# OpenDrift/opendrift

Measured on AMD Instinct MI355X. Metric: particle-steps/sec (RK4, 3D interp), higher is better.
Workload: dtype f64; 1 GPU; C3: OceanDrift 3D, synthetic ROMS-shaped z-level grid 1024x1024x12 (u,v,w,K), RK4 + vertical_mixing(60 s) + vertical_advection; particles_per_gpu=10000000, particles_total=10000000, stage_math=fast, spin_up_steps=200, block_every=0, inputs=resident in HBM, parallelism=particle-sharded x1, field block broadcast once per time level

## Files before the change

### include/odrift.h

```cpp
#ifndef ODRIFT_H
#define ODRIFT_H
#include <stdint.h>

#ifdef __cplusplus
extern "C" {
#endif

typedef struct odr_ctx odr_ctx;
typedef struct odr_particles odr_particles;

typedef enum {
  ODR_OK = 0,
  ODR_ERR_INVALID = -1,
  ODR_ERR_HIP = -2,
  ODR_ERR_CAPACITY = -3,
  ODR_ERR_STATE = -4
} odr_status;

enum {
  ODR_VAR_X_SEA_WATER_VELOCITY = 0,
  ODR_VAR_Y_SEA_WATER_VELOCITY = 1,
  ODR_VAR_X_WIND = 2,
  ODR_VAR_Y_WIND = 3,
  ODR_VAR_UPWARD_SEA_WATER_VELOCITY = 4,
// ... 243 lines not shown
  double layer_thick, particle_diameter, dissolved_diameter, diameter_uncertainty, desorption_depth, desorption_depth_uncert,
      resuspension_depth, resuspension_depth_uncert, resuspension_critvel;
} odr_radio_setup;
typedef struct odr_radio odr_radio;
int odr_radio_create(odr_ctx *ctx, const odr_radio_setup *setup, odr_radio **out);
int odr_radio_counts(odr_ctx *ctx, odr_radio *radio, int64_t *counts49, int reset);
int odr_radio_destroy(odr_ctx *ctx, odr_radio *radio);
int odr_radio_speciation(odr_ctx *ctx, odr_particles *p, odr_radio *radio, int specie_slot, int diameter_slot, int32_t conc3_var,
                         double dt_seconds, int rng_mode, const double *u1, const double *u2, const double *diameter_noise,
                         const double *depth_noise, uint64_t step);
int odr_radio_terminal_velocity(odr_ctx *ctx, odr_particles *p, int diameter_slot, int density_slot);
int odr_radio_resuspend(odr_ctx *ctx, odr_particles *p, odr_radio *radio, int specie_slot, int diameter_slot, int rng_mode,
                        const double *diameter_noise, const double *depth_noise, uint64_t step);
int odr_particles_count_status(odr_ctx *ctx, odr_particles *p, int32_t status_code, int64_t *n);
int odr_particles_remap_status(odr_ctx *ctx, odr_particles *p, int32_t from_code, int32_t to_code);
int odr_deactivate(odr_ctx *ctx, odr_particles *p, const uint8_t *mask_host, int32_t status_code);
int odr_deactivate_outside(odr_ctx *ctx, odr_particles *p, double west, double east, double south, double north,
                           int32_t status_code);
int odr_compact(odr_ctx *ctx, odr_particles *p, int64_t *n_active);
int odr_scan_status(odr_ctx *ctx, odr_particles *p, int64_t *n_kept, uint64_t *status_flags);
int odr_scan_status_begin(odr_ctx *ctx, odr_particles *p);
int odr_scan_status_end(odr_ctx *ctx, odr_particles *p, int64_t *n_kept, uint64_t *status_flags);
int odr_ctx_guard_next_vmix(odr_ctx *ctx, int on);
int odr_compact_apply(odr_ctx *ctx, odr_particles *p, int64_t *n_active);
int odr_sort_particles(odr_ctx *ctx, odr_particles *p, int32_t source_id);
int odr_sort_particles_ex(odr_ctx *ctx, odr_particles *p, int32_t source_id, int keep_environment);
int odr_particles_tile_stats(odr_ctx *ctx, odr_particles *p, uint64_t *out4);
int odr_particles_step_layout_stats(odr_ctx *ctx, odr_particles *p, uint64_t *out2);
int odr_particles_step_onlevel_stats(odr_ctx *ctx, odr_particles *p, uint64_t *out1);
int odr_particles_vmix_layout_stats(odr_ctx *ctx, odr_particles *p, uint64_t *out3);
int odr_particles_vmix_kplane_stats(odr_ctx *ctx, odr_particles *p, uint64_t *out2);
int odr_particles_vmix_window_stats(odr_ctx *ctx, odr_particles *p, uint64_t *out3);
int odr_particles_vmix_skip_stats(odr_ctx *ctx, odr_particles *p, uint64_t *out2);
int odr_reduce_scalars(odr_ctx *ctx, odr_particles *p, double wind_drift_depth, double *out16);
int odr_ctx_set_step_reduce(odr_ctx *ctx, int on, double wind_drift_depth, int relative_wind);
int odr_reduce_local(odr_ctx *ctx, odr_particles *p, double wind_drift_depth, int relative_wind, double *out16);
int odr_reduce_install(odr_ctx *ctx, odr_particles *p, const double *in16);
int odr_reduce_unpin(odr_ctx *ctx);

int odr_ctx_set_position_class(odr_ctx *ctx, int f32);
int odr_source_set_coordinate_dtype(odr_ctx *ctx, int32_t source_id, int x_is_float32, int y_is_float32);

#define ODR_COMM_ID_BYTES 256
int odr_device_count(int32_t *n);
int odr_comm_unique_id(uint8_t *id );
int odr_comm_init(odr_ctx *ctx, const uint8_t *id, int32_t rank, int32_t nranks);
int odr_comm_info(int32_t *rank, int32_t *nranks, uint64_t *id_hash, int32_t *rccl_version, uint64_t *collectives);
int odr_comm_destroy(void);
int odr_allreduce_scalars(odr_ctx *ctx, double *values, int32_t n, int32_t op);
int odr_comm_allgather_begin(odr_ctx *ctx, const double *row, int32_t n, int32_t from_scan);
int odr_comm_allgather_end(odr_ctx *ctx, double *rows );
int odr_comm_broadcast_bytes(odr_ctx *ctx, void *buf, int64_t nbytes, int32_t root);
int odr_comm_barrier(odr_ctx *ctx);
int odr_block_broadcast(odr_ctx *ctx, int32_t source_id, int32_t slot, double t_epoch, int nvars, const int32_t *var_ids,
                        const void *const *data, const int32_t *var_nz, int ny, int nx, const double *xy8, int32_t root);

int odr_timer_begin(odr_ctx *ctx);
int odr_timer_end(odr_ctx *ctx, float *ms);

enum {
  ODR_HIST_LON = 1000, ODR_HIST_LAT, ODR_HIST_Z, ODR_HIST_STATUS, ODR_HIST_MOVING, ODR_HIST_AGE_SECONDS,
  ODR_HIST_WIND_DRIFT_FACTOR, ODR_HIST_CURRENT_DRIFT_FACTOR, ODR_HIST_TERMINAL_VELOCITY,
  ODR_HIST_PROPERTY0 = 2000
};
typedef struct odr_history odr_history;
int odr_history_create(odr_ctx *ctx, int64_t n_trajectories, int32_t n_times, int32_t nvars,
// ... 97 lines not shown
```

### opendrift_amd/_abi.py

```python
import ctypes as C
import os

HERE = os.path.dirname(os.path.abspath(__file__))
LIB_PATH = os.environ.get('ODR_LIB') or os.path.join(HERE, 'libodrift_hip.so')

NVAR = 26
VARIABLES = {
    'x_sea_water_velocity': 0, 'y_sea_water_velocity': 1, 'x_wind': 2, 'y_wind': 3,
    'upward_sea_water_velocity': 4, 'ocean_vertical_diffusivity': 5,
    'sea_surface_wave_stokes_drift_x_velocity': 6, 'sea_surface_wave_stokes_drift_y_velocity': 7,
    'land_binary_mask': 8, 'sea_floor_depth_below_sea_level': 9, 'sea_surface_height': 10,
    'horizontal_diffusivity': 11, 'sea_surface_wave_significant_height': 12,
    'sea_surface_wave_period_at_variance_spectral_density_maximum': 13,
    'ocean_mixed_layer_thickness': 14,
    'sea_water_temperature': 15, 'sea_water_salinity': 16,
    'sea_ice_area_fraction': 17, 'sea_ice_x_velocity': 18, 'sea_ice_y_velocity': 19,
    'sea_surface_swell_wave_to_direction': 20,
    'sea_surface_swell_wave_peak_period_from_variance_spectral_density': 21,
    'sea_surface_swell_wave_significant_height': 22, 'sea_surface_wind_wave_to_direction': 23,
    'sea_surface_wind_wave_mean_period': 24, 'sea_surface_wind_wave_significant_height': 25,
}
VARIABLE_NAMES = {v: k for k, v in VARIABLES.items()}
PROJ_LATLONG, PROJ_STERE_EQUIT_SPHERE, PROJ_STERE_POLAR = 0, 1, 2
PROJ_MERC, PROJ_LCC = 4, 5
# ... 149 lines not shown
    'odr_particles_count_status': [_vp, _vp, C.c_int32, _i64p],
    'odr_particles_remap_status': [_vp, _vp, C.c_int32, C.c_int32],
    'odr_deactivate': [_vp, _vp, _P(C.c_uint8), C.c_int32],
    'odr_deactivate_outside': [_vp, _vp, C.c_double, C.c_double, C.c_double, C.c_double, C.c_int32],
    'odr_compact': [_vp, _vp, _i64p],
    'odr_vmix_set_profile_levels': [_vp, C.c_int32],
    'odr_ctx_set_position_class': [_vp, C.c_int],
    'odr_source_set_coordinate_dtype': [_vp, C.c_int32, C.c_int, C.c_int],
    'odr_device_count': [_P(C.c_int32)],
    'odr_comm_unique_id': [_P(C.c_uint8)],
    'odr_comm_init': [_vp, _P(C.c_uint8), C.c_int32, C.c_int32],
    'odr_comm_info': [_P(C.c_int32), _P(C.c_int32), _P(C.c_uint64), _P(C.c_int32), _P(C.c_uint64)],
    'odr_comm_destroy': [],
    'odr_allreduce_scalars': [_vp, _dp, C.c_int32, C.c_int32],
    'odr_comm_allgather_begin': [_vp, _dp, C.c_int32, C.c_int32],
    'odr_comm_allgather_end': [_vp, _dp],
    'odr_comm_broadcast_bytes': [_vp, _vp, C.c_int64, C.c_int32],
    'odr_comm_barrier': [_vp],
    'odr_block_broadcast': [_vp, C.c_int32, C.c_int32, C.c_double, C.c_int, _ip, _P(_vp), _ip, C.c_int, C.c_int, _dp, C.c_int32],
    'odr_scan_status': [_vp, _vp, _i64p, _P(C.c_uint64)],
    'odr_scan_status_begin': [_vp, _vp],
    'odr_scan_status_end': [_vp, _vp, _i64p, _P(C.c_uint64)],
    'odr_ctx_guard_next_vmix': [_vp, C.c_int],
    'odr_compact_apply': [_vp, _vp, _i64p],
    'odr_sort_particles': [_vp, _vp, C.c_int32],
    'odr_sort_particles_ex': [_vp, _vp, C.c_int32, C.c_int],
    'odr_particles_tile_stats': [_vp, _vp, _P(C.c_uint64)],
    'odr_particles_step_layout_stats': [_vp, _vp, _P(C.c_uint64)],
    'odr_particles_step_onlevel_stats': [_vp, _vp, _P(C.c_uint64)],
    'odr_particles_vmix_layout_stats': [_vp, _vp, _P(C.c_uint64)],
    'odr_particles_vmix_kplane_stats': [_vp, _vp, _P(C.c_uint64)],
    'odr_particles_vmix_window_stats': [_vp, _vp, _P(C.c_uint64)],
    'odr_particles_vmix_skip_stats': [_vp, _vp, _P(C.c_uint64)],
    'odr_reduce_scalars': [_vp, _vp, C.c_double, _dp],
    'odr_ctx_set_step_reduce': [_vp, C.c_int, C.c_double, C.c_int],
    'odr_reduce_local': [_vp, _vp, C.c_double, C.c_int, _dp],
    'odr_reduce_install': [_vp, _vp, _dp],
    'odr_reduce_unpin': [_vp],
    'odr_timer_begin': [_vp],
    'odr_timer_end': [_vp, _fp],
    'odr_sgrid_create': [_vp, C.c_int32, C.c_int32, C.c_int32, _dp, _dp, C.c_double, _dp, _dp, C.c_int32, _P(_vp)],
    'odr_sgrid_destroy': [_vp, _vp],
    'odr_sgrid_download_zrho': [_vp, _vp, _dp],
    'odr_sgrid_zslice': [_vp, _vp, _vp, C.c_int, C.c_int, C.c_int32, _dp, C.c_int32, _P(_vp), _dp],
    'odr_history_create': [_vp, C.c_int64, C.c_int32, C.c_int32, _ip, _P(_vp)],
    'odr_history_destroy': [_vp, _vp],
    'odr_history_set_id_base': [_vp, _vp, C.c_int64],
    'odr_history_record': [_vp, _vp, _vp, C.c_int32, C.c_int, C.c_int],
    'odr_history_flush': [_vp, _vp, C.c_int32, C.c_int32],
    'odr_history_wait': [_vp, _vp],
    'odr_history_host_ptr': [_vp, _vp, C.c_int32, _P(_fp), _P(C.c_int32)],
    'odr_history_reset': [_vp, _vp],
    'odr_history_minmax': [_vp, _vp, C.c_int32, _dp, _dp],
    'odr_density_map': [_vp, C.c_int64, C.c_int32] + [_vp] * 5 + [C.c_int32, C.c_int32, _dp, C.c_int32, _dp, _dp, _dp, _dp],
    'odr_density_last_kernel_ms': [_vp, _fp],
    'odr_density_map_proj': [_vp, C.c_int64, C.c_int32] + [_vp] * 5 + [C.c_int32, _P(ProjDesc), C.c_int32, _dp, C.c_int32, _dp, C.c_int64, _dp, _dp, _dp],
    'odr_species_layer_map': [_vp, C.c_int64, C.c_int32] + [_vp] * 4 + [_P(ProjDesc), C.c_int32, _dp, C.c_int32, _dp, C.c_int32, _dp, C.c_int32, _dp],
    'odr_conc_last_kernel_ms': [_vp, _fp],
    'odr_proj_extent': [_vp, _P(ProjDesc), C.c_int64, _vp, _vp, _dp],
    'odr_proj_grid_lonlat': [_vp, _P(ProjDesc), C.c_int32, _dp, C.c_int32, _dp, _dp, _dp],
    'odr_box_smooth': [_vp, C.c_int64, C.c_int32, C.c_int32, C.c_int32, _dp, _dp],
    'odr_ftle_map': [_vp, _P(ProjDesc), C.c_int32, C.c_int32, _dp, _dp, C.c_double, C.c_double, _vp, _vp, _fp, _dp],
    'odr_ftle_last_kernel_ms': [_vp, _fp],
    'odr_geod_inverse': [_vp, C.c_int64, _dp, _dp, _dp, _dp, _dp, _dp, _dp],
    'odr_trajectory_lengths': [_vp, C.c_int64, C.c_int32, _vp, _vp, C.c_double, _dp, _dp, _dp],
    'odr_trajectory_lengths_last_kernel_ms': [_vp, _fp],
# ... 71 lines not shown
```

### opendrift_amd/csrc/odr_host.h

```cpp
#pragma once
#include <hip/hip_runtime.h>

#include <algorithm>
#include <cmath>
#include <cstdarg>
#include <cstdio>
#include <cstdlib>
#include <cstring>
#include <initializer_list>
#include <string>
#include <vector>

#include "../../include/odrift.h"
#include "odr_kernels.hip.h"

using namespace odr;

#include <chrono>
struct SlowSpan {
  const char *what;
  std::chrono::steady_clock::time_point t0;
  static double limit() { static const double v = getenv("ODR_SLOW_CALLS") ? atof(getenv("ODR_SLOW_CALLS")) : 0.0; return v; }
  explicit SlowSpan(const char *w) : what(w) { if (limit() > 0) t0 = std::chrono::steady_clock::now(); }
  ~SlowSpan() {
// ... 99 lines not shown
  float *env[NVAR];
  float *altenv[NVAR];
  float *aux[9];
  float *altaux[9];
  bool profiles_f32 = false;
  unsigned aux_user = 0;
  bool kmember_on = false;
  float *aux_snap[9];
  long long aux_snap_cap[9];
  double *dead64[3];
  int *deadi32[2];
  unsigned *bcount;
  unsigned *wcount;
  unsigned long long wcount_epoch;
  long long wcount_n;
  void *scratch;
  size_t scratch_bytes;
  unsigned long long epoch;
  unsigned long long status_epoch, scan_epoch;
  long long scan_kept;
  float env_cval[NVAR];
  long long env_cn[NVAR];
  bool env_cok[NVAR];
  bool external;
  unsigned *wg_tab, *wg_list;
  unsigned long long *wg_total, *wg_stats;
  long long wg_cap, wg_grid, wg_n, wg_list_cap;
  unsigned long long wg_launches;
  unsigned long long step_launches[3];
  unsigned long long vmix_launches[3];
  unsigned long long vmix_kplane[2];
  unsigned long long vmix_window[2];
  unsigned long long vmix_tiled;
  unsigned long long *vmix_redone;
  double *z_keep;
  long long z_keep_n;
  bool z_truncated;
  int wg_sid;
  bool wg_valid;
  unsigned wg_src_gen;
};

static inline unsigned nblk(long long n) { return (unsigned)((n + BLOCK - 1) / BLOCK); }

static inline PView view(const odr_particles *p) {
  PView v;
  v.n = p->n;
  v.lon = p->d64[0]; v.lat = p->d64[1]; v.z = p->d64[2]; v.plon = p->d64[3]; v.plat = p->d64[4];
  v.slon = p->d64[5]; v.slat = p->d64[6];
  v.id = p->i32[0]; v.status = p->i32[1]; v.moving = p->i32[2];
  v.wdf = p->f32[0]; v.cdf = p->f32[1]; v.tv = p->f32[2]; v.age = p->f32[3];
  for (int k = 0; k < NVAR; ++k) v.env[k] = p->env[k];
  for (int k = 0; k < 9; ++k) v.aux[k] = p->aux[k];
  v.ice = p->ice_kind; v.pad = 0;
  v.rank = p->rank_on && p->rank ? p->rank : nullptr;
  return v;
}

static inline EnvGroupDesc env_bind_out(const EnvGroupDesc &G0, const PView &v) {
  EnvGroupDesc G = G0;
  for (int k = 0; k < MAXG; ++k) G.out_ptr[k] = k < G.nv ? v.env[G.var[k]] : nullptr;
  return G;
}

int flush_world(odr_ctx *c);
int flush_world_init(odr_ctx *c);

// ... 169 lines not shown
```

### opendrift_amd/csrc/odr_kernels.hip.h

```cpp
#pragma once
#include <hip/hip_runtime.h>
#include <rocrand/rocrand_kernel.h>
#include "odr_field.hip.h"

namespace odr {

#ifndef ODR_BLOCK
#define ODR_BLOCK 256
#endif
constexpr int BLOCK = ODR_BLOCK;
#ifndef ODR_POLAR_WAVES
#define ODR_POLAR_WAVES 3
#endif
#ifndef ODR_POLAR_STEP_WAVES
#define ODR_POLAR_STEP_WAVES 2
#endif
#define ODR_STEP_WAVES(PROJ) ((PROJ) == PROJ_LATLONG ? ODR_LATLONG_WAVES : ((PROJ) == PROJ_EXT ? 1 : ODR_POLAR_STEP_WAVES))
#ifndef ODR_LATLONG_WAVES
#define ODR_LATLONG_WAVES 1
#endif
#define ODR_WAVES(PROJ) ((PROJ) == PROJ_LATLONG ? ODR_LATLONG_WAVES : ((PROJ) == PROJ_EXT ? 1 : ODR_POLAR_WAVES))

__device__ __forceinline__ unsigned pid_wg() {
  const unsigned nb = gridDim.x, b = blockIdx.x, per = nb >> 3, rem = nb & 7u, x = b & 7u, j = b >> 3;
  return x * per + (x < rem ? x : rem) + j;
}
__device__ __forceinline__ long long pid() { return (long long)pid_wg() * BLOCK + threadIdx.x; }

struct PView {
  long long n;
  double *lon, *lat, *z, *plon, *plat;
  double *slon, *slat;
  int *id, *status, *moving;
  float *wdf, *cdf, *tv, *age;
  float *aux[9];
  float *env[NVAR];
  int ice;
  int pad;
  const int *rank;
};

__device__ __forceinline__ int sf_species_flag(const PView &p, int sfl, long long i) {
  if ((sfl & 255) != 5) return 0;
  const int sp = (int)p.aux[(sfl >> 24) & 15][i];
  return (sp >= 0 && sp < 7 && (((sfl >> 8) >> sp) & 1)) ? 8 : 0;
}

__device__ __forceinline__ float ice_k(float A) {
  float k = __fdiv_rn(__fsub_rn(A, 0.3f), 0.5f);
  if (A < 0.3f) k = 0.f;
  if (A > 0.8f) k = 1.f;
  return k;
}
__device__ __forceinline__ float ice_stokes_factor(float A) {
  float f = __fdiv_rn(__fsub_rn(0.7f, A), 0.7f);
  if (A > 0.7f) f = 0.f;
  return f;
}
__device__ __forceinline__ float current_factor(const PView &p, long long i, float factor) {
// ... 1768 lines not shown
    Dp.wgt = vmix_per_pass(D.wgt); Dp.Kfb = vmix_per_pass(D.Kfb);
    VMixArgs A;
    A.dt = vmix_per_pass(dt); A.dt_mix_cfg = vmix_per_pass(dt_mix_cfg);
    A.mix_at_surface = mix_at_surface; A.rng_mode = rng_mode; A.sfl = sfl; A.pad = 0;
    A.huni = huni; A.seed = seed; A.step = step;
    int t;
    asm volatile("v_mbcnt_lo_u32_b32 %0, -1, 0\n\tv_mbcnt_hi_u32_b32 %0, -1, %0" : "=&v"(t));
    t += (int)wave0;
    const unsigned e = e0 + (unsigned)t;
    long long i = 0;
    bool escaped = false;
    if (e < total) {
      i = base + list[e];
      long long i1 = i;
      asm volatile("" : "+v"(i1));
      const VMixState S = vmix_load_state(p, i1);
      escaped = vmix_col_particle<NQ, TL, VM>(s, p, Dp, A, vadv, i, Kp, gsh, t, S);
    }
    if constexpr (VM::WINDOW) {
      const unsigned long long esc = __ballot(escaped);
      if (esc != 0ull) {
        if (escaped) {
          long long i2 = i;
          asm volatile("" : "+v"(i2));
          const VMixState S2 = vmix_load_state(p, i2);
          vmix_col_particle<NQ, TL, typename VM::Full>(s, p, Dp, A, vadv, i, Kp, gsh, t, S2);
          if (D.redone && (t & 63) == __ffsll((long long)esc) - 1) atomicAdd(D.redone, (unsigned long long)__popcll(esc));
        }
      }
    }
  }
}

#ifndef ODR_VWIN_WAVES
#define ODR_VWIN_WAVES 5
#endif
template <bool TL>
__device__ __forceinline__ double vmix_layer(float b00, float b01, float b10, float b11, float a00, float a01, float a10, float a11,
                                             double w00, double w01, double w10, double w11, double wgt, bool cov, double Kfb) {
  double v = (double)bilw(b00, b01, b10, b11, w00, w01, w10, w11);
  if (TL) {
    const double w = (double)bilw(a00, a01, a10, a11, w00, w01, w10, w11);
    v = __dadd_rn(__dmul_rn(v, 1 - wgt), __dmul_rn(w, wgt));
  }
  return (cov && isfinite(v)) ? v : Kfb;
}
struct VMixGrad { double gd0, gi0, gd1, gi1, gd2, gi2, dt_mix; bool uniform_z; };
__device__ __forceinline__ void vmix_terms(const VMixGrad &G, const double *gsh, int nzp, int zl, double Kl, double Kz, double Kh,
                                           double &dk_dt, double &sg) {
  const double r = 1.0 / 3, ir = 1.0 / r;
  double gK;
  if (zl == 0) gK = div_cr(Kh - Kz, G.gd0, G.gi0);
  else if (zl == nzp - 1) gK = div_cr(Kz - Kl, G.gd1, G.gi1);
  else if (G.uniform_z) gK = div_cr(Kh - Kl, G.gd2, G.gi2);
  else gK = __dadd_rn(__dadd_rn(__dmul_rn(gsh[zl], Kl), __dmul_rn(gsh[nzp + zl], Kz)), __dmul_rn(gsh[2 * nzp + zl], Kh));
  double dK = -gK;
  if (fabs(dK) < 1e-10) dK = 0;
  dk_dt = __dmul_rn(dK, G.dt_mix);
  sg = sqrt(div_cr(__dmul_rn(__dmul_rn(Kz, fabs(G.dt_mix)), 2.0), r, ir));
}
template <bool TL>
__global__ __launch_bounds__(BLOCK, ODR_VWIN_WAVES) void k_vmix_win(const DevWorld *__restrict__ W, PView p, VMixDesc D,
                                                    double dt, double dt_mix_cfg, int mix_at_surface,
                                                    int rng_mode, const double *__restrict__ huni,
                                                    unsigned long long seed, unsigned long long step,
                                                    int vadv, int sfl) {
// ... 1436 lines not shown
```

### opendrift_amd/csrc/odr_mix.hip

```cpp
#define ODR_TU_MIX 1
#include "odr_host.h"

static_assert(vmix_col_lds_bytes(3) <= 163840 / ODR_VMIX_WAVES, "k_vmix_col<3>: column, tables and offset list exceed a sixth of the LDS");

template <class VM>
static bool vmix_layout_matches(const DevSource &s, const VMixDesc &D, int nq, double dt, double dt_mix, int mix_at_surface,
                                int rng_mode, int sfl, int vadv) {
  const bool uz = s.vg_uniform != 0;
  const int ntimes = abs((int)(dt / (dt_mix * (dt > 0 ? 1.0 : (dt < 0 ? -1.0 : 0.0)))));
  return VM::proj_kind(s.proj.kind) == s.proj.kind && VM::lon_mode(s.lon_mode) == s.lon_mode &&
         VM::mod360_x(s.mod360_x) == s.mod360_x && VM::nzp(D.nzp, 4 * nq) == D.nzp && VM::uniform_z(uz) == uz &&
         VM::rng_mode(rng_mode) == rng_mode && VM::mix_at_surface(mix_at_surface) == mix_at_surface &&
         VM::sf_action(sfl & 255) == (sfl & 255) && VM::vadv(vadv) == vadv && VM::ntimes(ntimes) == ntimes &&
         VM::kstride(D.kstride, nq) == D.kstride;
}

int odr_vmix(odr_ctx *c, odr_particles *p, double t, double dt, double dt_mix, int mix_at_surface, int rng_mode,
             const double *huni, uint64_t step) {
  const bool guarded = c->guard_next_vmix != 0;
  c->guard_next_vmix = 0;
  const bool oil = c->oil_owner == p;
  const bool f32prof = p->profiles_f32;
  const int cut = c->vmix_levels;
  VMixDesc D;
  bool kplanes = !getenv("ODR_NO_KPLANE");
  const bool fast = !oil && !f32prof && cut <= 0 && !getenv("ODR_NO_FAST_PATH") && build_vmix_desc(c, t, D, kplanes);
  if (guarded && (rng_mode == ODR_RNG_HOST || !fast)) return 1;
  const int vadv = c->fuse_vadv;
  c->fuse_vadv = -1;
  c->oil_owner = nullptr;
  c->vmix_levels = 0;
  c->guarded_vmix = nullptr;
  p->status_epoch++;
  p->epoch++;
  REQUIRE(dt_mix > 0 && dt != 0, "bad time steps");
  if (!p->env[VAR_DEPTH]) return fail(ODR_ERR_STATE, "sea_floor_depth_below_sea_level has not been sampled");
// ... 22 lines not shown
  dim3 g(nblk(p->n)), b(BLOCK);
  PView v = view(p);
  unsigned long long st = (unsigned long long)step;
  if (vadv >= 0 && !p->env[VAR_W]) return fail(ODR_ERR_STATE, "upward_sea_water_velocity has not been sampled");
  struct F32ProfileClass {
    odr_ctx *c;
    bool on;
    ~F32ProfileClass() { if (on) { c->hw.f32pos &= ~2; c->dirty = true; } }
  } f32bit{c, false};
  if (f32prof) { c->hw.f32pos |= 2; c->dirty = true; f32bit.on = true; if ((rc = flush_world(c))) return rc; }
  if (cut > 0) {
    REQUIRE(cut >= 2 && cut <= 255, "odr_vmix_set_profile_levels: 2 .. 255 levels");
    if (cut < nzp) nzp = cut;
  }
  const int sfl_cut = c->seafloor | ((cut > 0 ? nzp : 0) << 16);
  if (fast) {
    if (guarded) { D.guard = c->counter + 4; c->guarded_vmix = p; c->guarded_vadv = vadv; }
    const int nq = (nzp + 3) / 4;
    const bool tl = D.ka != nullptr;
    const char *wenv = getenv("ODR_VMIX_WINDOW");
    const bool win = nzp >= 3 && nzp <= BLOCK && (wenv ? atoi(wenv) != 0 : nzp > 12);
    const bool spec = !win && (nq == 2 || nq == 3) &&
                      vmix_layout_matches<VMixC3Rec>(c->hw.src[D.sid], D, nq, dt, dt_mix, mix_at_surface, rng_mode, c->seafloor, vadv) &&
                      !getenv("ODR_NO_VMIX_SPEC");
    const bool specp = spec && vmix_layout_matches<VMixC3>(c->hw.src[D.sid], D, nq, dt, dt_mix, mix_at_surface, rng_mode, c->seafloor, vadv);
    const bool quadwin = spec && nq == 3 && !getenv("ODR_NO_VMIX_WINDOW");
    p->vmix_launches[win ? 2 : spec ? 1 : 0]++;
    p->vmix_kplane[kplanes ? 0 : 1]++;
    if (spec && nq == 3) p->vmix_window[quadwin ? 0 : 1]++;
    D.redone = quadwin ? p->vmix_redone : nullptr;
    D.skipped = p->vmix_redone + 1;
    D.noskip = getenv("ODR_NO_VMIX_SKIP") ? 1 : 0;
    if (!win) { g = dim3((unsigned)((p->n + VMIX_TILE - 1) / VMIX_TILE)); p->vmix_tiled++; }
#define VMIX_COL(NQ, VM)                                                                                          \
  do {                                                                                                            \
    const size_t l2 = vmix_col_lds_bytes(NQ);                                                                     \
    if (tl) hipLaunchKernelGGL((k_vmix_col<NQ, true, VM>), g, b, l2, c->stream, c->dw, v, D, dt, dt_mix,          \
                               mix_at_surface, rng_mode, du, c->seed, st, vadv, c->seafloor);                                  \
    else hipLaunchKernelGGL((k_vmix_col<NQ, false, VM>), g, b, l2, c->stream, c->dw, v, D, dt, dt_mix,            \
                            mix_at_surface, rng_mode, du, c->seed, st, vadv, c->seafloor);                                     \
  } while (0)
    if (win) {
      const size_t lw = (sizeof(double) + sizeof(unsigned)) * 4 * BLOCK + sizeof(double) * 4 * (size_t)nzp;
      if (tl) hipLaunchKernelGGL((k_vmix_win<true>), g, b, lw, c->stream, c->dw, v, D, dt, dt_mix, mix_at_surface, rng_mode, du,
                                 c->seed, st, vadv, c->seafloor);
      else hipLaunchKernelGGL((k_vmix_win<false>), g, b, lw, c->stream, c->dw, v, D, dt, dt_mix, mix_at_surface, rng_mode, du,
                              c->seed, st, vadv, c->seafloor);
    }
    else if (specp && nq == 2) VMIX_COL(2, VMixC3);
    else if (specp && quadwin) VMIX_COL(3, VMixC3W);
    else if (specp) VMIX_COL(3, VMixC3);
    else if (spec && nq == 2) VMIX_COL(2, VMixC3Rec);
    else if (spec && quadwin) VMIX_COL(3, VMixC3RecW);
    else if (spec) VMIX_COL(3, VMixC3Rec);
    else if (nq <= 1) VMIX_COL(1, VMixRT);
    else if (nq == 2) VMIX_COL(2, VMixRT);
    else if (nq == 3) VMIX_COL(3, VMixRT);
    else if (nq == 4) VMIX_COL(4, VMixRT);
    else if (nq <= 6) VMIX_COL(6, VMixRT);
    else if (nq <= 8) VMIX_COL(8, VMixRT);
    else if (nq <= 12) VMIX_COL(12, VMixRT);
    else VMIX_COL(16, VMixRT);
#undef VMIX_COL
  } else if (oil) {
    if (nzp <= 16) hipLaunchKernelGGL((k_vmix<16, true>), g, b, lds, c->stream, c->dw, v, t, dt, dt_mix, mix_at_surface, rng_mode, du, c->seed, st, vadv, sfl_cut, c->oil);
    else if (nzp <= 32) hipLaunchKernelGGL((k_vmix<32, true>), g, b, lds, c->stream, c->dw, v, t, dt, dt_mix, mix_at_surface, rng_mode, du, c->seed, st, vadv, sfl_cut, c->oil);
    else hipLaunchKernelGGL((k_vmix<1, true>), g, b, lds, c->stream, c->dw, v, t, dt, dt_mix, mix_at_surface, rng_mode, du, c->seed, st, vadv, sfl_cut, c->oil);
  } else if (nzp <= 16) hipLaunchKernelGGL(k_vmix<16>, g, b, lds, c->stream, c->dw, v, t, dt, dt_mix, mix_at_surface, rng_mode, du, c->seed, st, vadv, sfl_cut);
  else if (nzp <= 32) hipLaunchKernelGGL(k_vmix<32>, g, b, lds, c->stream, c->dw, v, t, dt, dt_mix, mix_at_surface, rng_mode, du, c->seed, st, vadv, sfl_cut);
  else hipLaunchKernelGGL(k_vmix<1>, g, b, lds, c->stream, c->dw, v, t, dt, dt_mix, mix_at_surface, rng_mode, du, c->seed, st, vadv, sfl_cut);
  if (!fast) p->vmix_launches[2]++;
  HIPCHK(hipGetLastError());
  return 0;
}

int odr_particles_vmix_layout_stats(odr_ctx *c, odr_particles *p, uint64_t *out3) {
  REQUIRE(c && p && out3, "NULL argument");
  for (int k = 0; k < 3; ++k) out3[k] = p->vmix_launches[k];
  return 0;
}

int odr_particles_vmix_kplane_stats(odr_ctx *c, odr_particles *p, uint64_t *out2) {
  REQUIRE(c && p && out2, "NULL argument");
  out2[0] = p->vmix_kplane[0]; out2[1] = p->vmix_kplane[1];
  return 0;
}

int odr_particles_vmix_skip_stats(odr_ctx *c, odr_particles *p, uint64_t *out2) {
  REQUIRE(c && p && out2, "NULL argument");
  unsigned long long skipped = 0;
  D2H(&skipped, p->vmix_redone + 1, sizeof skipped);
  HIPCHK(hipStreamSynchronize(c->stream));
  out2[0] = p->vmix_tiled; out2[1] = skipped;
  return 0;
}

int odr_particles_vmix_window_stats(odr_ctx *c, odr_particles *p, uint64_t *out3) {
  REQUIRE(c && p && out3, "NULL argument");
  unsigned long long redone = 0;
  D2H(&redone, p->vmix_redone, sizeof redone);
  HIPCHK(hipStreamSynchronize(c->stream));
  out3[0] = p->vmix_window[0]; out3[1] = p->vmix_window[1]; out3[2] = redone;
  return 0;
}

int odr_vmix_set_profile_levels(odr_ctx *c, int32_t n) {
  REQUIRE(n == 0 || (n >= 2 && n <= 255), "bad level count %d", n);
  c->vmix_levels = n;
  return 0;
}

int odr_vmix_wind_profile(odr_ctx *c, odr_particles *p, int model, double background_diffusivity, double dt,
                          double dt_mix, int mix_at_surface, int rng_mode, const double *huni, uint64_t step) {
  c->guard_next_vmix = 0;
  p->status_epoch++;
  p->epoch++;
  REQUIRE(model == ODR_DIFFUSIVITY_LARGE1994 || model == ODR_DIFFUSIVITY_SUNDBY1983, "Unknown diffusivity model: %d", model);
  REQUIRE(dt_mix > 0 && dt != 0, "bad time steps");
  if (!p->env[VAR_DEPTH]) return fail(ODR_ERR_STATE, "sea_floor_depth_below_sea_level has not been sampled");
  int rc;
  if ((rc = seafloor_species_slot_ok(c, p))) return rc;
  for (int v : {VAR_SSH, VAR_XWIND, VAR_YWIND, VAR_MLD})
    if ((rc = ensure_env(c, p, v))) return rc;
  if ((rc = flush_world(c))) return rc;
  if (p->n == 0) return 0;
  p->epoch++;
// ... 161 lines not shown
```

### opendrift_amd/csrc/odrift.hip

```cpp
#define ODR_TU_MISC 1
#include "odr_host.h"
#include "odr_mesh.h"

static thread_local std::string g_err;
int odr_i_fail(int code, const char *fmt, ...) {
  char buf[512];
  va_list ap;
  va_start(ap, fmt);
  vsnprintf(buf, sizeof buf, fmt, ap);
  va_end(ap);
  g_err = buf;
  return code;
}

const char *odr_last_error(void) { return g_err.c_str(); }
#define ODR_STR2(x) #x
#define ODR_STR(x) ODR_STR2(x)
const char *odr_version(void) { return "odrift-hip 0.2 (gfx950; mixing stream Philox4x32-" ODR_STR(ODR_MIX_ROUNDS) ")"; }

int odr_ctx_create(int device, uint64_t seed, odr_ctx **out) {
  REQUIRE(out, "out is NULL");
  HIPCHK(hipSetDevice(device));
  odr_ctx *c = new odr_ctx();
  c->device = device;
// ... 69 lines not shown
}

int odr_set_stream(odr_ctx *c, void *s) {
  HIPCHK(hipStreamSynchronize(c->stream));
  c->stream = s ? (hipStream_t)s : c->own_stream;
  return 0;
}

int odr_timer_begin(odr_ctx *c) {
  HIPCHK(hipEventRecord(c->ev0, c->stream));
  return 0;
}
int odr_timer_end(odr_ctx *c, float *ms) {
  HIPCHK(hipEventRecord(c->ev1, c->stream));
  HIPCHK(hipEventSynchronize(c->ev1));
  HIPCHK(hipEventElapsedTime(ms, c->ev0, c->ev1));
  return 0;
}

int odr_particles_create(odr_ctx *c, int64_t capacity, odr_particles **out) {
  REQUIRE(capacity > 0 && out, "capacity must be positive");
  HIPCHK(hipSetDevice(c->device));
  odr_particles *p = new odr_particles();
  memset(p, 0, sizeof(*p));
  p->cap = capacity;
  p->dead_cap = capacity;
  p->scan_kept = -1;
  for (int k = 0; k < 7; ++k) HIPCHK(hipMalloc((void **)&p->d64[k], sizeof(double) * (size_t)capacity));
  for (int k = 0; k < 3; ++k) HIPCHK(hipMalloc((void **)&p->i32[k], sizeof(int) * (size_t)capacity));
  for (int k = 0; k < 4; ++k) HIPCHK(hipMalloc((void **)&p->f32[k], sizeof(float) * (size_t)capacity));
  HIPCHK(hipMalloc((void **)&p->bcount, sizeof(unsigned) * (size_t)(nblk(capacity) + 1)));
  HIPCHK(hipMalloc((void **)&p->wcount, sizeof(unsigned) * (size_t)(nblk(capacity) + 1) * (BLOCK / 64)));
  p->wcount_epoch = ~0ull;
  HIPCHK(hipMalloc((void **)&p->vmix_redone, 2 * sizeof(unsigned long long)));
  HIPCHK(hipMemset(p->vmix_redone, 0, 2 * sizeof(unsigned long long)));
  *out = p;
  return 0;
}

int odr_particles_destroy(odr_ctx *c, odr_particles *p) {
  if (c->red_owner == p) c->red_owner = nullptr;
  if (c->noise_owner == p) c->noise_owner = nullptr;
  if (c->guarded_vmix == p) c->guarded_vmix = nullptr;
  if (!p) return 0;
  (void)hipStreamSynchronize(c->stream);
  auto fr = [](void *q) { if (q) (void)hipFree(q); };
  for (int k = 0; k < 7; ++k) { fr(p->d64[k]); fr(p->alt64[k]); }
  for (int k = 0; k < 3; ++k) { fr(p->i32[k]); fr(p->alti32[k]); fr(p->dead64[k]); }
  for (int k = 0; k < 4; ++k) { fr(p->f32[k]); fr(p->altf32[k]); }
  for (int k = 0; k < 2; ++k) fr(p->deadi32[k]);
  for (int k = 0; k < NVAR; ++k) { fr(p->env[k]); fr(p->altenv[k]); }
  for (int k = 0; k < 9; ++k) { fr(p->aux[k]); fr(p->altaux[k]); fr(p->aux_snap[k]); }
  fr(p->bcount);
  fr(p->wcount);
  fr(p->vmix_redone);
  fr(p->scratch);
  fr(p->rank); fr(p->rank_words); fr(p->rank_before); fr(p->rank_bsum);
  fr(p->wg_tab); fr(p->wg_total); fr(p->wg_list); fr(p->z_keep);
  delete p;
  return 0;
}

template <class T>
static int put(odr_ctx *c, T *dst, const T *src, long long n, T dflt) {
  if (src) {
    H2D(dst, src, sizeof(T) * (size_t)n);
  } else {
    std::vector<T> tmp((size_t)n, dflt);
    H2D(dst, tmp.data(), sizeof(T) * (size_t)n);
    HIPCHK(hipStreamSynchronize(c->stream));
  }
  return 0;
}

int odr_particles_append(odr_ctx *c, odr_particles *p, int64_t n, const double *lon, const double *lat,
                         const double *z, const int32_t *id, const int32_t *moving, const float *wdf,
                         const float *cdf, const float *tv) {
  p->status_epoch++;
  p->epoch++;
  REQUIRE(n >= 0 && lon && lat, "lon/lat required");
  if (p->n + n > p->cap) return fail(ODR_ERR_CAPACITY, "capacity %lld exceeded (%lld + %lld)", p->cap, p->n, (long long)n);
  if (n == 0) return 0;
  long long o = p->n;
  int rc;
  if ((rc = put<double>(c, p->d64[0] + o, lon, n, 0.0))) return rc;
  if ((rc = put<double>(c, p->d64[1] + o, lat, n, 0.0))) return rc;
  if ((rc = put<double>(c, p->d64[2] + o, z, n, 0.0))) return rc;
  if ((rc = put<double>(c, p->d64[3] + o, lon, n, 0.0))) return rc;
// ... 2400 lines not shown
```

### opendrift_amd/device.py

```python
import ctypes as C
import os

import numpy as np

from . import _abi
from ._abi import VARIABLES, check

_dp, _fp, _ip = C.POINTER(C.c_double), C.POINTER(C.c_float), C.POINTER(C.c_int32)


def _vid(v, aliases=None):
    if isinstance(v, (int, np.integer)):
        return v
    if v in VARIABLES:
        return VARIABLES[v]
    if aliases and v in aliases:
        return aliases[v]
    raise KeyError(v)


def _d(a, n=None):
    if a is None:
        return None, None
    a = np.ascontiguousarray(np.broadcast_to(np.asarray(a, dtype=np.float64), (n,)) if n is not None
# ... 1173 lines not shown
        check(self.lib.odr_particles_step_layout_stats(self.ctx.h, self.h, out))
        return dict(runtime=int(out[0]), static=int(out[1]))

    def step_onlevel_stats(self):
        import ctypes as C
        out = (C.c_uint64 * 1)()
        check(self.lib.odr_particles_step_onlevel_stats(self.ctx.h, self.h, out))
        return int(out[0])

    def vmix_layout_stats(self):
        import ctypes as C
        out = (C.c_uint64 * 3)()
        check(self.lib.odr_particles_vmix_layout_stats(self.ctx.h, self.h, out))
        return dict(runtime=int(out[0]), static=int(out[1]), other=int(out[2]))

    def vmix_kplane_stats(self):
        import ctypes as C
        out = (C.c_uint64 * 2)()
        check(self.lib.odr_particles_vmix_kplane_stats(self.ctx.h, self.h, out))
        return dict(planes=int(out[0]), records=int(out[1]))

    def vmix_window_stats(self):
        import ctypes as C
        out = (C.c_uint64 * 3)()
        check(self.lib.odr_particles_vmix_window_stats(self.ctx.h, self.h, out))
        return dict(windowed=int(out[0]), full=int(out[1]), redone=int(out[2]))

    def vmix_skip_stats(self):
        import ctypes as C
        out = (C.c_uint64 * 2)()
        check(self.lib.odr_particles_vmix_skip_stats(self.ctx.h, self.h, out))
        return dict(launches=int(out[0]), skipped=int(out[1]))

    def reduce_global(self, combine, wind_drift_depth=0.1, relative_wind=False):
        raw = np.empty(16)
        check(self.lib.odr_reduce_local(self.ctx.h, self.h, float(wind_drift_depth), int(relative_wind), raw.ctypes.data_as(_dp)))
        g = np.ascontiguousarray(combine(raw), dtype=np.float64)
        check(self.lib.odr_reduce_install(self.ctx.h, self.h, g.ctypes.data_as(_dp)))
        return g

    def reduce_local(self, wind_drift_depth=0.1, relative_wind=False):
        raw = np.empty(16)
        check(self.lib.odr_reduce_local(self.ctx.h, self.h, float(wind_drift_depth), int(relative_wind), raw.ctypes.data_as(_dp)))
        return raw

    def reduce_install(self, combined16):
        g = np.ascontiguousarray(combined16, dtype=np.float64)
        check(self.lib.odr_reduce_install(self.ctx.h, self.h, g.ctypes.data_as(_dp)))

    @staticmethod
    def reduction_dict(raw):
        keys = ['n_active', 'lon_min', 'lon_max', 'lat_min', 'lat_max', 'z_min', 'z_max', 'D_max',
                'stokes_sum_max', 'wind_speed_max', 'wdf_surface_max', 'n_surface', 'hs_max', 'tp_max']
        d = dict(zip(keys, raw))
        for k in ('lon_min', 'lat_min', 'z_min'):
            d[k] = -d[k]
        return d

    def reduce_unpin(self):
        check(self.lib.odr_reduce_unpin(self.ctx.h))

    def reduce_scalars(self, wind_drift_depth=0.1):
        out = np.empty(16)
        check(self.lib.odr_reduce_scalars(self.ctx.h, self.h, float(wind_drift_depth), out.ctypes.data_as(_dp)))
        keys = ['n_active', 'lon_min', 'lon_max', 'lat_min', 'lat_max', 'z_min', 'z_max', 'D_max',
                'stokes_sum_max', 'wind_speed_max', 'wdf_surface_max', 'n_surface', 'hs_max', 'tp_max']
# ... 334 lines not shown
```

Baseline: 11.94 billion particle-steps/s.

## Compact vertical-mixing work into a dense list of non-skipped particles

Adds a three-kernel pre-pass (ballot keep mask per tile, single-block prefix scan, list fill) that builds a compacted index list of particles that actually need vertical mixing. A new dense vmix kernel then launches over only those particles, so no wave is spent on surface particles that would be skipped. The cost is three extra launches, extra mask/list memory, a serial single-block scan, and indirect (gathered) particle access in the mixing kernel.

```diff
diff --git a/include/odrift.h b/include/odrift.h
--- a/include/odrift.h
+++ b/include/odrift.h
@@ -299,6 +299,7 @@
 int odr_particles_vmix_kplane_stats(odr_ctx *ctx, odr_particles *p, uint64_t *out2);
 int odr_particles_vmix_window_stats(odr_ctx *ctx, odr_particles *p, uint64_t *out3);
 int odr_particles_vmix_skip_stats(odr_ctx *ctx, odr_particles *p, uint64_t *out2);
+int odr_particles_vmix_dense_stats(odr_ctx *ctx, odr_particles *p, uint64_t *out2);
 int odr_reduce_scalars(odr_ctx *ctx, odr_particles *p, double wind_drift_depth, double *out16);
 int odr_ctx_set_step_reduce(odr_ctx *ctx, int on, double wind_drift_depth, int relative_wind);
 int odr_reduce_local(odr_ctx *ctx, odr_particles *p, double wind_drift_depth, int relative_wind, double *out16);
diff --git a/opendrift_amd/_abi.py b/opendrift_amd/_abi.py
--- a/opendrift_amd/_abi.py
+++ b/opendrift_amd/_abi.py
@@ -205,6 +205,7 @@
     'odr_particles_vmix_kplane_stats': [_vp, _vp, _P(C.c_uint64)],
     'odr_particles_vmix_window_stats': [_vp, _vp, _P(C.c_uint64)],
     'odr_particles_vmix_skip_stats': [_vp, _vp, _P(C.c_uint64)],
+    'odr_particles_vmix_dense_stats': [_vp, _vp, _P(C.c_uint64)],
     'odr_reduce_scalars': [_vp, _vp, C.c_double, _dp],
     'odr_ctx_set_step_reduce': [_vp, C.c_int, C.c_double, C.c_int],
     'odr_reduce_local': [_vp, _vp, C.c_double, C.c_int, _dp],
diff --git a/opendrift_amd/csrc/odr_host.h b/opendrift_amd/csrc/odr_host.h
--- a/opendrift_amd/csrc/odr_host.h
+++ b/opendrift_amd/csrc/odr_host.h
@@ -155,7 +155,10 @@
   unsigned long long vmix_kplane[2];
   unsigned long long vmix_window[2];
   unsigned long long vmix_tiled;
+  unsigned long long vmix_dense;
   unsigned long long *vmix_redone;
+  unsigned long long *vmix_mask;
+  unsigned *vmix_toff, *vmix_list;
   double *z_keep;
   long long z_keep_n;
   bool z_truncated;
diff --git a/opendrift_amd/csrc/odr_kernels.hip.h b/opendrift_amd/csrc/odr_kernels.hip.h
--- a/opendrift_amd/csrc/odr_kernels.hip.h
+++ b/opendrift_amd/csrc/odr_kernels.hip.h
@@ -21,10 +21,11 @@
 #endif
 #define ODR_WAVES(PROJ) ((PROJ) == PROJ_LATLONG ? ODR_LATLONG_WAVES : ((PROJ) == PROJ_EXT ? 1 : ODR_POLAR_WAVES))
 
-__device__ __forceinline__ unsigned pid_wg() {
-  const unsigned nb = gridDim.x, b = blockIdx.x, per = nb >> 3, rem = nb & 7u, x = b & 7u, j = b >> 3;
+__device__ __forceinline__ unsigned pid_wg_of(unsigned nb) {
+  const unsigned b = blockIdx.x, per = nb >> 3, rem = nb & 7u, x = b & 7u, j = b >> 3;
   return x * per + (x < rem ? x : rem) + j;
 }
+__device__ __forceinline__ unsigned pid_wg() { return pid_wg_of(gridDim.x); }
 __device__ __forceinline__ long long pid() { return (long long)pid_wg() * BLOCK + threadIdx.x; }
 
 struct PView {
@@ -1859,6 +1860,172 @@
   }
 }
 
+struct VMixKeep {
+  unsigned long long *mask;
+  unsigned *toff;
+  unsigned *list;
+  unsigned *hdr;
+  unsigned long long *listed;
+};
+__global__ __launch_bounds__(BLOCK) void k_vmix_keep(PView p, VMixKeep K, const unsigned long long *guard, double dt,
+                                                      double dt_mix_cfg) {
+  if (guard && *guard == 0ull) return;
+  constexpr int NW = BLOCK / 64;
+  __shared__ unsigned cnt[NW];
+  const int tid = threadIdx.x, lane = tid & 63, wave = tid >> 6;
+  const long long base = (long long)blockIdx.x * VMIX_TILE;
+  double z[VMIX_TILE_ROUNDS];
+  float dep[VMIX_TILE_ROUNDS], ssh[VMIX_TILE_ROUNDS];
+#pragma unroll
+  for (int r = 0; r < VMIX_TILE_ROUNDS; ++r) {
+    const long long e = base + r * BLOCK + tid, ec = e < p.n ? e : 0;
+    z[r] = p.z[ec]; dep[r] = p.env[VAR_DEPTH][ec]; ssh[r] = p.env[VAR_SSH][ec];
+  }
+  const double sgn = dt > 0 ? 1.0 : (dt < 0 ? -1.0 : 0.0);
+  const bool walks = abs((int)(dt / (dt_mix_cfg * sgn))) > 0;
+  unsigned mine = 0;
+#pragma unroll
+  for (int r = 0; r < VMIX_TILE_ROUNDS; ++r) {
+    const long long e = base + r * BLOCK + tid;
+    const float Zmin = __fmul_rn(-1.f, __fadd_rn(dep[r], ssh[r]));
+    const bool skip = e < p.n && z[r] == 0 && !(Zmin > 0.f);
+    if (skip && walks && __double_as_longlong(z[r]) != 0ll) p.z[e] = 0.0;
+    const unsigned long long keep = __ballot(e < p.n && !skip);
+    if (lane == 0) K.mask[(size_t)blockIdx.x * (VMIX_TILE / 64) + r * NW + wave] = keep;
+    mine += (unsigned)__popcll(keep);
+  }
+  if (lane == 0) cnt[wave] = mine;
+  __syncthreads();
+  if (tid == 0) {
+    unsigned t = 0;
+#pragma unroll
+    for (int w = 0; w < NW; ++w) t += cnt[w];
+    K.toff[blockIdx.x] = t;
+  }
+}
+constexpr int VMIX_SCAN_ROWS = 16;
+__global__ __launch_bounds__(1024) void k_vmix_keep_scan(VMixKeep K, long long ntiles, long long n,
+                                                          const unsigned long long *guard, unsigned long long *skipped) {
+  const int tid = threadIdx.x, lane = tid & 63, wv = tid >> 6;
+  if (guard && *guard == 0ull) {
+    if (tid == 0) { K.hdr[0] = 0u; K.hdr[1] = 0u; }
+    return;
+  }
+  constexpr int G = VMIX_SCAN_ROWS;
+  __shared__ unsigned wtot[G * 16];
+  unsigned carry = 0;
+  for (long long k0 = 0; k0 < ntiles; k0 += (long long)G * 1024) {
+    unsigned v[G], x[G];
+#pragma unroll
+    for (int u = 0; u < G; ++u) {
+      const long long k = k0 + (long long)u * 1024 + tid;
+      v[u] = k < ntiles ? K.toff[k] : 0u;
+    }
+#pragma unroll
+    for (int u = 0; u < G; ++u) {
+      x[u] = v[u];
+#pragma unroll
+      for (int o = 1; o < 64; o <<= 1) { const unsigned y = __shfl_up(x[u], o, 64); if (lane >= o) x[u] += y; }
+      if (lane == 63) wtot[u * 16 + wv] = x[u];
+    }
+    __syncthreads();
+    if (wv == 0) {
+#pragma unroll
+      for (int b0 = 0; b0 < G * 16; b0 += 64) {
+        const unsigned t0 = wtot[b0 + lane];
+        unsigned s = t0;
+#pragma unroll
+        for (int o = 1; o < 64; o <<= 1) { const unsigned y = __shfl_up(s, o, 64); if (lane >= o) s += y; }
+        wtot[b0 + lane] = carry + s - t0;
+        carry += __shfl(s, 63, 64);
+      }
+    }
+    __syncthreads();
+#pragma unroll
+    for (int u = 0; u < G; ++u) {
+      const long long k = k0 + (long long)u * 1024 + tid;
+      if (k < ntiles) K.toff[k] = x[u] - v[u] + wtot[u * 16 + wv];
+    }
+    __syncthreads();
+  }
+  if (tid == 0) {
+    K.hdr[0] = carry;
+    K.hdr[1] = (carry + (unsigned)BLOCK - 1u) / (unsigned)BLOCK;
+    if (skipped && (unsigned long long)n > carry) atomicAdd(skipped, (unsigned long long)n - carry);
+    if (carry) atomicAdd(K.listed, (unsigned long long)carry);
+  }
+}
+__global__ __launch_bounds__(BLOCK) void k_vmix_keep_fill(VMixKeep K, const unsigned long long *guard) {
+  if (guard && *guard == 0ull) return;
+  constexpr int NW = BLOCK / 64;
+  const int tid = threadIdx.x, lane = tid & 63;
+  const int wave = __builtin_amdgcn_readfirstlane(tid >> 6);
+  const unsigned long long *m = K.mask + (size_t)blockIdx.x * (VMIX_TILE / 64);
+  unsigned run = K.toff[blockIdx.x], off[VMIX_TILE_ROUNDS];
+  unsigned long long keep[VMIX_TILE_ROUNDS];
+#pragma unroll
+  for (int g = 0; g < VMIX_TILE / 64; ++g) {
+    const unsigned long long mg = m[g];
+    if ((g % NW) == wave) { off[g / NW] = run; keep[g / NW] = mg; }
+    run += (unsigned)__popcll(mg);
+  }
+  const unsigned long long below = (1ull << lane) - 1ull;
+  const unsigned first = (unsigned)blockIdx.x * (unsigned)VMIX_TILE;
+#pragma unroll
+  for (int r = 0; r < VMIX_TILE_ROUNDS; ++r)
+    if ((keep[r] >> lane) & 1ull) K.list[off[r] + (unsigned)__popcll(keep[r] & below)] = first + (unsigned)(r * BLOCK + tid);
+}
+__host__ __device__ constexpr size_t vmix_dense_lds_bytes(int nq) {
+  return sizeof(double) * ((size_t)(4 * nq) * BLOCK + 4 * (size_t)(4 * nq));
+}
+template <int NQ, bool TL, class VM>
+__global__ __launch_bounds__(BLOCK, ODR_VMIX_WAVES) void k_vmix_dense(const DevWorld *__restrict__ W, PView p, VMixDesc D,
+                                                      const unsigned *__restrict__ list, const unsigned *__restrict__ hdr,
+                                                      double dt, double dt_mix_cfg, int mix_at_surface,
+                                                      int rng_mode, const double *__restrict__ huni,
+                                                      unsigned long long seed, unsigned long long step,
+                                                      int vadv, int sfl) {
+  static_assert(VM::STATIC, "the dense launch exists for the static configurations");
+  constexpr int NL = 4 * NQ;
+  extern __shared__ __attribute__((aligned(16))) char smem[];
+  const int tid = threadIdx.x;
+  const DevSource &s = W->src[D.sid];
+  const int nzp = VM::nzp(D.nzp, NL);
+  double *Kp = (double *)smem;
+  double *gsh = Kp + (size_t)NL * BLOCK;
+  if (D.guard && *D.guard == 0ull) return;
+  const unsigned total = hdr[0], nbd = hdr[1];
+  if (blockIdx.x >= nbd) return;
+  const unsigned d = pid_wg_of(nbd) * BLOCK + (unsigned)tid;
+  const bool valid = d < total;
+  const long long i = list[valid ? d : 0u];
+  if (tid < nzp) {
+    gsh[tid] = s.vg_a[tid]; gsh[NL + tid] = s.vg_b[tid]; gsh[2 * NL + tid] = s.vg_c[tid];
+    gsh[3 * NL + tid] = s.zmid[tid];
+  }
+  long long i1 = i;
+  asm volatile("" : "+v"(i1));
+  const VMixState S = vmix_load_state(p, i1);
+  __syncthreads();
+  if (!valid) return;
+  VMixArgs A;
+  A.dt = dt; A.dt_mix_cfg = dt_mix_cfg; A.mix_at_surface = mix_at_surface; A.rng_mode = rng_mode; A.sfl = sfl; A.pad = 0;
+  A.huni = huni; A.seed = seed; A.step = step;
+  const bool escaped = vmix_col_particle<NQ, TL, VM>(s, p, D, A, vadv, i, Kp, gsh, tid, S);
+  if constexpr (VM::WINDOW) {
+    const unsigned long long esc = __ballot(escaped);
+    if (esc != 0ull) {
+      if (escaped) {
+        long long i2 = i;
+        asm volatile("" : "+v"(i2));
+        const VMixState S2 = vmix_load_state(p, i2);
+        vmix_col_particle<NQ, TL, typename VM::Full>(s, p, D, A, vadv, i, Kp, gsh, tid, S2);
+        if (D.redone && (tid & 63) == __ffsll((long long)esc) - 1) atomicAdd(D.redone, (unsigned long long)__popcll(esc));
+      }
+    }
+  }
+}
+
 #ifndef ODR_VWIN_WAVES
 #define ODR_VWIN_WAVES 5
 #endif
diff --git a/opendrift_amd/csrc/odr_mix.hip b/opendrift_amd/csrc/odr_mix.hip
--- a/opendrift_amd/csrc/odr_mix.hip
+++ b/opendrift_amd/csrc/odr_mix.hip
@@ -2,6 +2,8 @@
 #include "odr_host.h"
 
 static_assert(vmix_col_lds_bytes(3) <= 163840 / ODR_VMIX_WAVES, "k_vmix_col<3>: column, tables and offset list exceed a sixth of the LDS");
+static_assert(vmix_dense_lds_bytes(3) <= 163840 / ODR_VMIX_WAVES, "k_vmix_dense<3>: column and tables exceed a sixth of the LDS");
+static_assert(VMIX_TILE == 1024, "odr_particles_create sizes the keep ballots and tile counts for tiles of 1024 elements");
 
 template <class VM>
 static bool vmix_layout_matches(const DevSource &s, const VMixDesc &D, int nq, double dt, double dt_mix, int mix_at_surface,
@@ -90,6 +92,26 @@
     D.skipped = p->vmix_redone + 1;
     D.noskip = getenv("ODR_NO_VMIX_SKIP") ? 1 : 0;
     if (!win) { g = dim3((unsigned)((p->n + VMIX_TILE - 1) / VMIX_TILE)); p->vmix_tiled++; }
+    const bool dense = spec && mix_at_surface == 0 && vadv != 1 && !D.noskip && !getenv("ODR_NO_VMIX_DENSE") &&
+                       p->n <= 0xffffffffLL;
+    VMixKeep K;
+    K.mask = p->vmix_mask; K.toff = p->vmix_toff; K.list = p->vmix_list;
+    K.hdr = (unsigned *)(p->vmix_redone + 3); K.listed = p->vmix_redone + 2;
+    if (dense) {
+      hipLaunchKernelGGL(k_vmix_keep, g, b, 0, c->stream, v, K, D.guard, dt, dt_mix);
+      hipLaunchKernelGGL(k_vmix_keep_scan, dim3(1), dim3(1024), 0, c->stream, K, (long long)g.x, (long long)p->n, D.guard, D.skipped);
+      hipLaunchKernelGGL(k_vmix_keep_fill, g, b, 0, c->stream, K, D.guard);
+      g = dim3(nblk(p->n));
+      p->vmix_dense++;
+    }
+#define VMIX_DENSE(NQ, VM)                                                                                        \
+  do {                                                                                                            \
+    const size_t l2 = vmix_dense_lds_bytes(NQ);                                                                   \
+    if (tl) hipLaunchKernelGGL((k_vmix_dense<NQ, true, VM>), g, b, l2, c->stream, c->dw, v, D, K.list, K.hdr, dt, dt_mix, \
+                               mix_at_surface, rng_mode, du, c->seed, st, vadv, c->seafloor);                     \
+    else hipLaunchKernelGGL((k_vmix_dense<NQ, false, VM>), g, b, l2, c->stream, c->dw, v, D, K.list, K.hdr, dt, dt_mix, \
+                            mix_at_surface, rng_mode, du, c->seed, st, vadv, c->seafloor);                        \
+  } while (0)
 #define VMIX_COL(NQ, VM)                                                                                          \
   do {                                                                                                            \
     const size_t l2 = vmix_col_lds_bytes(NQ);                                                                     \
@@ -105,6 +127,12 @@
       else hipLaunchKernelGGL((k_vmix_win<false>), g, b, lw, c->stream, c->dw, v, D, dt, dt_mix, mix_at_surface, rng_mode, du,
                               c->seed, st, vadv, c->seafloor);
     }
+    else if (dense && specp && nq == 2) VMIX_DENSE(2, VMixC3);
+    else if (dense && specp && quadwin) VMIX_DENSE(3, VMixC3W);
+    else if (dense && specp) VMIX_DENSE(3, VMixC3);
+    else if (dense && nq == 2) VMIX_DENSE(2, VMixC3Rec);
+    else if (dense && quadwin) VMIX_DENSE(3, VMixC3RecW);
+    else if (dense) VMIX_DENSE(3, VMixC3Rec);
     else if (specp && nq == 2) VMIX_COL(2, VMixC3);
     else if (specp && quadwin) VMIX_COL(3, VMixC3W);
     else if (specp) VMIX_COL(3, VMixC3);
@@ -120,6 +148,7 @@
     else if (nq <= 12) VMIX_COL(12, VMixRT);
     else VMIX_COL(16, VMixRT);
 #undef VMIX_COL
+#undef VMIX_DENSE
   } else if (oil) {
     if (nzp <= 16) hipLaunchKernelGGL((k_vmix<16, true>), g, b, lds, c->stream, c->dw, v, t, dt, dt_mix, mix_at_surface, rng_mode, du, c->seed, st, vadv, sfl_cut, c->oil);
     else if (nzp <= 32) hipLaunchKernelGGL((k_vmix<32, true>), g, b, lds, c->stream, c->dw, v, t, dt, dt_mix, mix_at_surface, rng_mode, du, c->seed, st, vadv, sfl_cut, c->oil);
@@ -150,6 +179,15 @@
   D2H(&skipped, p->vmix_redone + 1, sizeof skipped);
   HIPCHK(hipStreamSynchronize(c->stream));
   out2[0] = p->vmix_tiled; out2[1] = skipped;
+  return 0;
+}
+
+int odr_particles_vmix_dense_stats(odr_ctx *c, odr_particles *p, uint64_t *out2) {
+  REQUIRE(c && p && out2, "NULL argument");
+  unsigned long long listed = 0;
+  D2H(&listed, p->vmix_redone + 2, sizeof listed);
+  HIPCHK(hipStreamSynchronize(c->stream));
+  out2[0] = p->vmix_dense; out2[1] = listed;
   return 0;
 }
 
diff --git a/opendrift_amd/csrc/odrift.hip b/opendrift_amd/csrc/odrift.hip
--- a/opendrift_amd/csrc/odrift.hip
+++ b/opendrift_amd/csrc/odrift.hip
@@ -125,8 +125,12 @@
   HIPCHK(hipMalloc((void **)&p->bcount, sizeof(unsigned) * (size_t)(nblk(capacity) + 1)));
   HIPCHK(hipMalloc((void **)&p->wcount, sizeof(unsigned) * (size_t)(nblk(capacity) + 1) * (BLOCK / 64)));
   p->wcount_epoch = ~0ull;
-  HIPCHK(hipMalloc((void **)&p->vmix_redone, 2 * sizeof(unsigned long long)));
-  HIPCHK(hipMemset(p->vmix_redone, 0, 2 * sizeof(unsigned long long)));
+  HIPCHK(hipMalloc((void **)&p->vmix_redone, 4 * sizeof(unsigned long long)));
+  HIPCHK(hipMemset(p->vmix_redone, 0, 4 * sizeof(unsigned long long)));
+  const size_t vtiles = ((size_t)capacity + 1023) / 1024;
+  HIPCHK(hipMalloc((void **)&p->vmix_mask, sizeof(unsigned long long) * 16 * vtiles));
+  HIPCHK(hipMalloc((void **)&p->vmix_toff, sizeof(unsigned) * vtiles));
+  HIPCHK(hipMalloc((void **)&p->vmix_list, sizeof(unsigned) * (size_t)capacity));
   *out = p;
   return 0;
 }
@@ -147,6 +151,7 @@
   fr(p->bcount);
   fr(p->wcount);
   fr(p->vmix_redone);
+  fr(p->vmix_mask); fr(p->vmix_toff); fr(p->vmix_list);
   fr(p->scratch);
   fr(p->rank); fr(p->rank_words); fr(p->rank_before); fr(p->rank_bsum);
   fr(p->wg_tab); fr(p->wg_total); fr(p->wg_list); fr(p->z_keep);
diff --git a/opendrift_amd/device.py b/opendrift_amd/device.py
--- a/opendrift_amd/device.py
+++ b/opendrift_amd/device.py
@@ -1229,6 +1229,12 @@
         check(self.lib.odr_particles_vmix_skip_stats(self.ctx.h, self.h, out))
         return dict(launches=int(out[0]), skipped=int(out[1]))
 
+    def vmix_dense_stats(self):
+        import ctypes as C
+        out = (C.c_uint64 * 2)()
+        check(self.lib.odr_particles_vmix_dense_stats(self.ctx.h, self.h, out))
+        return dict(launches=int(out[0]), listed=int(out[1]))
+
     def reduce_global(self, combine, wind_drift_depth=0.1, relative_wind=False):
         raw = np.empty(16)
         check(self.lib.odr_reduce_local(self.ctx.h, self.h, float(wind_drift_depth), int(relative_wind), raw.ctypes.data_as(_dp)))
```

New measurement: 12.16 billion particle-steps/s, median of 6. 1.9% higher.
